# sharph/s-rack

Measured on AMD Instinct MI355X. Metric: voice-samples/sec @48 kHz offline render, higher is better.
Workload: dtype f32

## Files before the change

s-rack_amd/csrc/chain.hip:

```cpp
#include "fused.hip.h"
#include "launch.hpp"

namespace srack {

__global__ __launch_bounds__(64) void render_ctl_gate_env(CtlWork w)
{
    if (w.port & OSC_EXACT)
        ctl_gate_env<true>(w);
    else
        ctl_gate_env<false>(w);
}

void launch_ctl_gate_env(const CtlWork& w, hipStream_t st)
{
    hipLaunchKernelGGL(render_ctl_gate_env, dim3(1), dim3(64), 0, st, w);
}

void launch_fused(uint32_t osc_port, uint32_t vcf_port, bool exact, int out_mode, bool track, const KernelArgs& ka, const ChainRoles& roles, const CtlWork& co,
                  dim3 grid, hipStream_t st)
{
    with_osc_port(osc_port, [&](auto A) { launch_chain<decltype(A)::value>(vcf_port, exact, out_mode, track, ka, roles, co, grid, st); });
}

}
```

s-rack_amd/csrc/fused.hip.h:

```cpp
#pragma once
#include <hip/hip_runtime.h>
#include <type_traits>

#include "kernel_args.hip.h"
#include "launch_types.hpp"
#include "modules.hip.h"
#include "wave.hip.h"

#ifndef SRK_PRIO_AT1
#define SRK_PRIO_AT1 32
#endif
#ifndef SRK_PRIO_AT0
#define SRK_PRIO_AT0 56
#endif


namespace srack {


template <uint32_t kOscPort, bool kExact>
SRK_DEV void ctl_gate_env_body(const CtlWork& a)
{
    using namespace dev;
    const ChainRoles r{0, 0, 0, 1, 0, 2, 0};
    const int lane = threadIdx.x;
    auto row = [&](int rr) { return a.table[rr]; };
    const DevOp& ol = a.ops[r.osc_l];
    const DevOp& od = a.ops[r.adsr];
    float* __restrict__ track = a.track;

    COsc cl;
    cosc_init(cl, make_f64(row(ol.state_row + OSC_S_POS_LO), row(ol.state_row + OSC_S_POS_HI)), ol.delta);
    AdsrRegs sd;
    sd.phase = __uint_as_float(row(od.state_row + ADSR_S_PHASE));
    sd.mode = (int)row(od.state_row + ADSR_S_MODE);
    sd.r_val = __uint_as_float(row(od.state_row + ADSR_S_R_VAL));
    sd.from_a_val = __uint_as_float(row(od.state_row + ADSR_S_FROM_A));
    sd.gate_last = row(od.state_row + ADSR_S_GATE_LAST) != 0;
    const AdsrConst kd = adsr_consts(od.par_val[ADSR_P_A], od.par_val[ADSR_P_D], od.par_val[ADSR_P_S], od.par_val[ADSR_P_R], od.par_val[ADSR_P_SR]);
    AdsrSeg seg;
    adsr_seg_enter(sd, kd, seg);

    constexpr uint32_t osc_flags = OSC_AA | kOscPort | (kExact ? OSC_EXACT : 0u);
    for (uint32_t t0 = 0; t0 < a.T; t0 += kMixRows) {
        const int n = (int)min((uint32_t)kMixRows, a.T - t0);
        const float gate = cosc_tile<kExact>(osc_flags, cl, n);
        const float env = adsr_seg_tile(sd, kd, seg, gate, n);
        if (lane < n) track[t0 + lane] = env;
    }
    adsr_seg_flush(sd, seg);
    uint32_t* const tout = a.table_out ? a.table_out : a.table;
    if (a.table_out) {
        for (uint32_t rr = (uint32_t)lane; rr < a.n_rows; rr += 64u) a.table_out[rr] = a.table[rr];
        __builtin_amdgcn_fence(__ATOMIC_RELEASE, "workgroup");
    }
    if (lane == 0) {
        tout[ol.state_row + OSC_S_POS_LO] = f64_lo(cl.pos);
        tout[ol.state_row + OSC_S_POS_HI] = f64_hi(cl.pos);
        tout[ol.state_row + OSC_S_SYNC_LAST] = 0u;
        tout[od.state_row + ADSR_S_PHASE] = __float_as_uint(sd.phase);
        tout[od.state_row + ADSR_S_MODE] = (uint32_t)sd.mode;
        tout[od.state_row + ADSR_S_R_VAL] = __float_as_uint(sd.r_val);
        tout[od.state_row + ADSR_S_FROM_A] = __float_as_uint(sd.from_a_val);
        tout[od.state_row + ADSR_S_GATE_LAST] = sd.gate_last ? 1u : 0u;
    }
}


template <bool kExact>
SRK_DEV void ctl_gate_env(const CtlWork& w)
{
    const uint32_t port = w.port & (OSC_OUT_SINE | OSC_OUT_SQUARE | OSC_OUT_SAW);
    if (port == OSC_OUT_SQUARE)
        ctl_gate_env_body<OSC_OUT_SQUARE, kExact>(w);
    else if (port == OSC_OUT_SAW)
        ctl_gate_env_body<OSC_OUT_SAW, kExact>(w);
    else
        ctl_gate_env_body<OSC_OUT_SINE, kExact>(w);
}


template <uint32_t kOscAPort, uint32_t kOscLPort, uint32_t kVcfPort, bool kExact, int kOut>
__global__ __launch_bounds__(64) void render_voice_chain(KernelArgs a, ChainRoles r)
{
    using namespace dev;
    __shared__ __attribute__((aligned(16))) float mix_tile[kMixTile];
    const int lane = threadIdx.x;
    const WaveMap wm = wave_map(a, lane);
    const uint32_t voice = wm.voice, vc = wm.vc, V = a.V;
    const bool active = wm.active;
    auto row = [&](int rr) { return a.table[(size_t)rr * V + vc]; };
    auto parv = [&](const DevOp& op, int k) { return op.par_row[k] >= 0 ? __uint_as_float(row(op.par_row[k])) : op.par_val[k]; };

    const DevOp& oa = a.ops[r.osc_a];
    const DevOp& ol = a.ops[r.osc_l];
    const DevOp& ov = a.ops[r.vcf];
    const DevOp& od = a.ops[r.adsr];
    const DevOp& oc = a.ops[r.vca];
    const int plane = a.ops[r.out].aux;

    constexpr uint32_t kEx = kExact ? OSC_EXACT : 0u;
    constexpr uint32_t fa = OSC_AA | kOscAPort | kEx;
    constexpr uint32_t fl = OSC_AA | kOscLPort | kEx;

    OscRegs sa, sl;
    OscConst ka, kl;
    sa.pos = make_f64(row(oa.state_row + OSC_S_POS_LO), row(oa.state_row + OSC_S_POS_HI));
    sa.sync_last = row(oa.state_row + OSC_S_SYNC_LAST) != 0;
    sl.pos = make_f64(row(ol.state_row + OSC_S_POS_LO), row(ol.state_row + OSC_S_POS_HI));
    sl.sync_last = row(ol.state_row + OSC_S_SYNC_LAST) != 0;
    ka.sr = oa.sample_rate;
    ka.val = 0.0;
    ka.delta = oa.delta_row >= 0 ? make_f64(row(oa.delta_row), row(oa.delta_row + 1)) : oa.delta;
    ka.inv_dt = inv_dt_f32(ka.delta);
    kl.sr = ol.sample_rate;
    kl.val = 0.0;
    kl.delta = ol.delta_row >= 0 ? make_f64(row(ol.delta_row), row(ol.delta_row + 1)) : ol.delta;
    kl.inv_dt = inv_dt_f32(kl.delta);

    VcfRegs sv;
    {
        const int s0 = ov.state_row;
        sv.f = __uint_as_float(row(s0 + VCF_S_F));
        sv.p = __uint_as_float(row(s0 + VCF_S_P));
        sv.q = __uint_as_float(row(s0 + VCF_S_Q));
        sv.b0 = __uint_as_float(row(s0 + VCF_S_B0 + 0));
        sv.b1 = __uint_as_float(row(s0 + VCF_S_B0 + 1));
        sv.b2 = __uint_as_float(row(s0 + VCF_S_B0 + 2));
        sv.b3 = __uint_as_float(row(s0 + VCF_S_B0 + 3));
        sv.b4 = __uint_as_float(row(s0 + VCF_S_B0 + 4));
        sv.freq = __uint_as_float(row(s0 + VCF_S_FREQ));
// ... 99 lines not shown
        put(s0 + VCF_S_P, __float_as_uint(sv.p));
        put(s0 + VCF_S_Q, __float_as_uint(sv.q));
        put(s0 + VCF_S_B0 + 0, __float_as_uint(sv.b0));
        put(s0 + VCF_S_B0 + 1, __float_as_uint(sv.b1));
        put(s0 + VCF_S_B0 + 2, __float_as_uint(sv.b2));
        put(s0 + VCF_S_B0 + 3, __float_as_uint(sv.b3));
        put(s0 + VCF_S_B0 + 4, __float_as_uint(sv.b4));
        put(s0 + VCF_S_FREQ, __float_as_uint(sv.freq));
        put(s0 + VCF_S_RES, __float_as_uint(sv.res));
        put(od.state_row + ADSR_S_PHASE, __float_as_uint(sd.phase));
        put(od.state_row + ADSR_S_MODE, (uint32_t)sd.mode);
        put(od.state_row + ADSR_S_R_VAL, __float_as_uint(sd.r_val));
        put(od.state_row + ADSR_S_FROM_A, __float_as_uint(sd.from_a_val));
        put(od.state_row + ADSR_S_GATE_LAST, sd.gate_last ? 1u : 0u);
    }
}

#ifdef SRK_WAVE_CENSUS
static __device__ uint32_t* srk_census_rec;
SRK_DEV uint32_t* census_begin(uint32_t slot, uint32_t wave, bool ctl, int lane)
{
    uint32_t* rec = srk_census_rec;
    if (!rec || lane != 0) return nullptr;
    rec += (size_t)slot * 8;
    const uint64_t t = __builtin_amdgcn_s_memrealtime();
    rec[0] = (uint32_t)t;
    rec[1] = (uint32_t)(t >> 32);
    rec[4] = (uint32_t)__builtin_amdgcn_s_getreg((31 << 11) | 4);
    rec[5] = (uint32_t)__builtin_amdgcn_s_getreg((31 << 11) | 20);
    rec[6] = ctl ? 3u : 1u;
    rec[7] = wave;
    return rec;
}
SRK_DEV void census_end(uint32_t* rec)
{
    if (!rec) return;
    const uint64_t t = __builtin_amdgcn_s_memrealtime();
    rec[2] = (uint32_t)t;
    rec[3] = (uint32_t)(t >> 32);
}
SRK_DEV void census_end(uint32_t* rec, const dev::Pace& p)
{
    if (rec && p.word) rec[6] = 1u | 4u | (p.key << 3) | ((p.max_lead < 255u ? p.max_lead : 255u) << 16) | ((p.mine < 255u ? p.mine : 255u) << 24);
    census_end(rec);
}
#endif

template <uint32_t kOscAPort, uint32_t kVcfPort, bool kExact, int kOut>
__global__ __launch_bounds__(64) void render_voice_chain_track(KernelArgs a, ChainRoles r, CtlWork co)
{
    using namespace dev;
    __shared__ __attribute__((aligned(16))) float mix_tile[kMixTile];
    if (blockIdx.x < a.block0) {
        __builtin_amdgcn_s_setprio(3);
#ifdef SRK_WAVE_CENSUS
        uint32_t* crec = census_begin(a.n_waves, 0xffffffffu, true, threadIdx.x);
#endif
        ctl_gate_env<kExact>(co);
#ifdef SRK_WAVE_CENSUS
        census_end(crec);
#endif
        return;
    }
    const int lane = threadIdx.x;
#ifdef SRK_WAVE_CENSUS
    uint32_t* crec = census_begin(blockIdx.x - a.block0, blockIdx.x - a.block0, false, lane);
#endif
    const WaveMap wm = wave_map(a, lane);
    const uint32_t voice = wm.voice, vc = wm.vc, V = a.V;
    const bool active = wm.active;
    auto row = [&](int rr) { return a.table[(size_t)rr * V + vc]; };
    auto parv = [&](const DevOp& op, int k) { return op.par_row[k] >= 0 ? __uint_as_float(row(op.par_row[k])) : op.par_val[k]; };

    const DevOp& oa = a.ops[r.osc_a];
    const DevOp& ov = a.ops[r.vcf];
    const DevOp& oc = a.ops[r.vca];
    const int plane = a.ops[r.out].aux;
    const float* __restrict__ env_track = a.tracks + (size_t)r.track * a.t_stride;

    constexpr uint32_t fa = OSC_AA | kOscAPort | (kExact ? OSC_EXACT : 0u);
    OscRegs sa;
    OscConst ka;
    sa.pos = make_f64(row(oa.state_row + OSC_S_POS_LO), row(oa.state_row + OSC_S_POS_HI));
    sa.sync_last = row(oa.state_row + OSC_S_SYNC_LAST) != 0;
    ka.sr = oa.sample_rate;
    ka.val = 0.0;
    ka.delta = oa.delta_row >= 0 ? make_f64(row(oa.delta_row), row(oa.delta_row + 1)) : oa.delta;
    ka.inv_dt = inv_dt_f32(ka.delta);

    VcfRegs sv;
    const int s0 = ov.state_row;
    sv.f = __uint_as_float(row(s0 + VCF_S_F));
    sv.p = __uint_as_float(row(s0 + VCF_S_P));
    sv.q = __uint_as_float(row(s0 + VCF_S_Q));
    sv.b0 = __uint_as_float(row(s0 + VCF_S_B0 + 0));
    sv.b1 = __uint_as_float(row(s0 + VCF_S_B0 + 1));
    sv.b2 = __uint_as_float(row(s0 + VCF_S_B0 + 2));
    sv.b3 = __uint_as_float(row(s0 + VCF_S_B0 + 3));
    sv.b4 = __uint_as_float(row(s0 + VCF_S_B0 + 4));
    sv.freq = __uint_as_float(row(s0 + VCF_S_FREQ));
    sv.res = __uint_as_float(row(s0 + VCF_S_RES));
    if (a.T > 0) vcf_coeffs<!kExact>(sv, vcf_frequency(parv(ov, VCF_P_FREQ), 0.0f, parv(ov, VCF_P_EXP)), vcf_resonance(parv(ov, VCF_P_RES)));
    bool sv_fin = !kExact || vcf_nan_free(sv);
    const bool negative = parv(oc, VCA_P_NEG) != 0.0f;

    EmitOf<kOut> em = make_emit_of<kOut>(a, plane, lane);

    constexpr bool kFixed = !kExact && kOscAPort == OSC_OUT_SAW;
    COsc ca;
    FOsc fa_osc;
    float x = 0.0f;
// ... 155 lines not shown
```

s-rack_amd/csrc/launch_types.hpp:

```cpp
#pragma once
#include <cstdint>

#include "kernel_args.hip.h"

namespace srack {

struct CtlWork {
    const DevOp* ops;
    uint32_t* table;
    float* track;
    uint32_t T;
    uint32_t port;
    uint32_t* table_out;
    uint32_t n_rows;
};

constexpr int kBlkVoices = 32, kBlkSlices = 16, kBlkPer = 16, kBlkChunk = kBlkSlices * kBlkPer;

struct MasterArgs {
    const float* rows;
    const float* gain;
    float* runs;
    float* master;
    double* stats;
    uint32_t n;
    uint32_t n_buses;
    uint32_t row_channels;
    uint32_t used;
};

struct SendRun {
    uint32_t dst;
    uint32_t first;
    uint32_t count;
    int32_t srow;
};
struct SendMulti {
    uint32_t dst;
    uint32_t first_row;
    uint32_t n_runs;
    uint32_t pad;
};
static_assert(sizeof(SendRun) == 16 && sizeof(SendMulti) == 16, "the host keeps both tables as four 32-bit words per entry (runtime.hpp)");
struct SendArgs {
    const float* rows;
    float* out;
    float* scratch;
    const uint32_t* term_src;
    const float* term_gain;
    const SendRun* runs;
    const SendMulti* multi;
    uint32_t n;
    uint32_t row_channels;
    uint32_t used;
    uint32_t n_runs;
    uint32_t n_multi;
    uint32_t max_blocks;
};

struct BusVcfRow {
    uint32_t row;
    uint32_t bus;
    uint32_t slot;
    uint32_t port;
    float freq, res, exp_amt;
    uint32_t pad;
};
// ... 71 lines not shown
```

s-rack_amd/csrc/modules.hip.h:

```cpp
#pragma once
#ifndef __HIPCC_RTC__
#include <hip/hip_runtime.h>
#endif

#ifdef __HIPCC_RTC__
#include "srack_hip.h"
#else
#include "../../include/srack_hip.h"
#endif
#include "program.hpp"

namespace srack {
namespace dev {

#define SRK_DEV __device__ __forceinline__

SRK_DEV float keep(float x)
{
    asm("" : "+v"(x));
    return x;
}

SRK_DEV float zero_f32()
{
// ... 710 lines not shown
    uint64_t near = __builtin_amdgcn_ballot_w64(h <= o.hA) | __builtin_amdgcn_ballot_w64(h >= o.hB);
    if (kPort == OSC_OUT_SQUARE) near |= __builtin_amdgcn_ballot_w64((uint32_t)(h - o.hQ0) <= o.hQspan);
    if (near != 0) {
        OscRegs g;
        g.pos = o.pos;
        g.sync_last = false;
        OscConst k;
        k.delta = o.delta;
        k.val = 0.0;
        k.sr = 0.0;
        k.inv_dt = 0.0f;
        float o3[3] = {0.0f, 0.0f, 0.0f};
        osc_step(OSC_AA | OSC_EXACT | kPort, g, k, 0.0f, 0.0f, o3[0], o3[1], o3[2]);
        o.pos = g.pos;
        return kPort == OSC_OUT_SQUARE ? o3[1] : o3[2];
    }
    const float y = kPort == OSC_OUT_SQUARE ? (h < 0x3fe00000 ? -1.0f : 1.0f) : (float)o.pos * 2.0f - 1.0f;
    o.pos = __builtin_amdgcn_fract(o.pos + o.delta);
    return y;
}

template <bool kExact>
SRK_DEV float cosc_tile(uint32_t flags, COsc& o, int n)
{
    const int lane = (int)(threadIdx.x & 63u);
    double pos = o.pos, mine = o.pos;
    const bool tame = !kExact || __builtin_amdgcn_ballot_w64(!(pos >= 0.0 && pos < 1.0 && o.delta >= 0.0 && o.delta < 1.0)) == 0;
    if (tame && n == kTileRows) {
#pragma unroll 8
        for (int j = 0; j < kTileRows; j++) {
            mine = lane == j ? pos : mine;
            pos = __builtin_amdgcn_fract(pos + o.delta);
        }
    } else {
        for (int j = 0; j < n; j++) {
            mine = lane == j ? pos : mine;
            pos = tame ? __builtin_amdgcn_fract(pos + o.delta) : fmod1(pos + o.delta);
        }
    }
    o.pos = pos;
    OscRegs g;
    g.pos = mine;
    g.sync_last = false;
    OscConst k;
    k.delta = o.delta;
    k.val = 0.0;
    k.sr = 0.0;
    k.inv_dt = o.inv_dt;
    float y0 = 0.0f, y1 = 0.0f, y2 = 0.0f;
    osc_step(flags, g, k, 0.0f, 0.0f, y0, y1, y2);
    return (flags & OSC_OUT_SAW) ? y2 : ((flags & OSC_OUT_SQUARE) ? y1 : y0);
}

struct StepOsc {
    COsc o;
    float seen_cv;
    bool carried;
};

SRK_DEV void steposc_init(StepOsc& s, double pos)
{
    s.o.pos = pos;
    s.o.delta = 0.0;
    s.seen_cv = __builtin_nanf("");
    s.carried = false;
}

template <uint32_t kPort>
SRK_DEV float steposc_step(StepOsc& s, const OscConst& k, float cv)
{
    COsc& o = s.o;
    if (__builtin_amdgcn_ballot_w64(cv != s.seen_cv) != 0) {
        const double delta = osc_delta_cold((double)cv + k.val, k.sr);
        s.seen_cv = cv;
        s.carried = __builtin_amdgcn_ballot_w64(!(delta < 0.25)) == 0;
        cosc_init(o, o.pos, delta);
    }
    if (s.carried) return cosc_step<kPort>(o);
    OscRegs g;
    g.pos = o.pos;
    g.sync_last = false;
    g.seen_cv = s.seen_cv;
    g.seen_delta = o.delta;
    float o3[3] = {0.0f, 0.0f, 0.0f};
    osc_step(OSC_HAS_CV | OSC_CV_STEPWISE | OSC_AA | kPort, g, k, cv, 0.0f, o3[0], o3[1], o3[2]);
    cosc_init(o, g.pos, o.delta);
    return kPort == OSC_OUT_SAW ? o3[2] : (kPort == OSC_OUT_SQUARE ? o3[1] : o3[0]);
}

struct FOsc {
    uint32_t lo, hi;
    uint32_t dlo, dhi;
    float c32;
    float ta;
    float inv_s;
    bool first;
};

SRK_DEV void fosc_init(FOsc& o, uint32_t lo, uint32_t hi, uint32_t dlo, uint32_t dhi)
{
    o.lo = lo;
    o.hi = hi;
    o.dlo = dlo;
    o.dhi = dhi;
    const double delta = __builtin_fma((double)dhi, 0x1p-32, (double)dlo * 0x1p-64);
    o.inv_s = inv_dt_f32(delta) * 0x1p-32f;
// ... 414 lines not shown
    const bool open = g.c0 >= 0.0f && g.c1 >= 0.0f && (g.c0 > 0.0f || (g.c1 > 1.0e-30f && u_first > 1.0e-6f)) && g.c0 < 1.0e30f && g.c1 < 1.0e30f;
    decided = open || closed;
    return open;
}
SRK_DEV float vca_step_decided(bool open_lane, float audio, float cv)
{
    const float y = audio * cv;
    return open_lane ? y : 0.0f;
}

SRK_DEV float adsr_seg_quiet_step(AdsrRegs& s, AdsrSeg& g)
{
    s.phase = s.phase + g.inc;
    const float u = __builtin_fmaf(g.k1, s.phase, g.k0);
    const float out = g.c0 + g.c1 * u;
    g.held = out;
    return out;
}

SRK_DEV float adsr_seg_tile(AdsrRegs& s, const AdsrConst& c, AdsrSeg& g, float gate, int n)
{
    const int lane = (int)(threadIdx.x & 63u);
    const uint64_t tile = (1ull << n) - 1ull;
    const uint64_t high = __builtin_amdgcn_ballot_w64(gate > 0.0f) & tile;
    const uint64_t before = (high << 1) | (g.last != 0 ? 1ull : 0ull);
    float keep = 0.0f;
    int i = 0;
    while (i < n) {
        const uint64_t ends = ((g.on_high != 0 ? high : 0ull) | (g.on_low != 0 ? ~high : 0ull) | (g.on_edge != 0 ? (high & ~before) : 0ull)) & tile & (~0ull << i);
        const int by_gate = ends != 0 ? (int)__builtin_ctzll(ends) : n;
        const float room = (0.9999f - s.phase) * __builtin_amdgcn_rcpf(g.inc);
        const int by_phase = __builtin_amdgcn_readfirstlane(room > 0.0f ? (int)__builtin_fminf(room, 64.0f) : 0);
        const int run = min(by_gate - i, by_phase);
        if (run > 0) {
            float ph = s.phase, out = g.held;
            for (int k = 0; k < run; k++) {
                ph = ph + g.inc;
                const float u = __builtin_fmaf(g.k1, ph, g.k0);
                out = g.c0 + g.c1 * u;
                keep = lane == i + k ? out : keep;
            }
            s.phase = ph;
            g.held = out;
            i += run;
            g.last = ((high >> (i - 1)) & 1ull) ? ~0ull : 0ull;
        }
        if (i < n) {
            const float y = adsr_seg_step(s, c, g, __int_as_float(__builtin_amdgcn_readlane(__float_as_int(gate), i)));
            keep = lane == i ? y : keep;
            i++;
        }
    }
    return keep;
}

SRK_DEV float vca_step(uint32_t flags, bool negative, float audio, float cv)
{
    if ((flags & (VCA_HAS_AUDIO | VCA_HAS_CV)) != (VCA_HAS_AUDIO | VCA_HAS_CV)) return zero_f32();
    return (negative || cv > 0.0f) ? audio * cv : 0.0f;
}

SRK_DEV float vca_step_uniform(uint32_t flags, bool negative, float audio, float cv)
{
    if ((flags & (VCA_HAS_AUDIO | VCA_HAS_CV)) != (VCA_HAS_AUDIO | VCA_HAS_CV)) return zero_f32();
    const bool cv_pos = (uint32_t)(__float_as_int(cv) - 1) < 0x7f800000u;
    return (negative || cv_pos) ? audio * cv : 0.0f;
}

SRK_DEV float mixer_step(uint32_t connected, const float in[4], const float gain[4])
{
    float out = zero_f32();
#pragma unroll
    for (int k = 0; k < 4; k++)
        if (connected & (1u << k)) out = out + in[k] * gain[k];
    return out;
}

SRK_DEV float math_step(uint32_t flags, float in1, float in2, float constant)
{
    float a = (flags & MATH_HAS_IN1) ? in1 : zero_f32();
    float b = (flags & MATH_HAS_IN2) ? in2 : constant;
    switch ((flags >> MATH_OP_SHIFT) & 3u) {
    case SRACK_MATH_ADD: return a + b;
    case SRACK_MATH_SUBTRACT: return a - b;
    default: return a * b;
    }
}

SRK_DEV uint64_t splitmix64(uint64_t x)
{
    x += 0x9E3779B97F4A7C15ull;
    x = (x ^ (x >> 30)) * 0xBF58476D1CE4E5B9ull;
    x = (x ^ (x >> 27)) * 0x94D049BB133111EBull;
    return x ^ (x >> 31);
}
SRK_DEV uint64_t noise_voice_key(uint64_t base, uint64_t global_voice) { return splitmix64(base ^ global_voice); }
SRK_DEV float noise_sample(uint64_t key, uint64_t n)
{
    const uint32_t k24 = (uint32_t)(splitmix64(key + n * 0x9E3779B97F4A7C15ull) >> 40);
    return ((float)k24 * 0x1p-24f - 0.5f) * 2.0f;
}

__device__ const uint64_t kPowfLog2Tab[16][2] = {
    {0x3ff661ec79f8f3be, 0xbfdefec65b963019}, {0x3ff571ed4aaf883d, 0xbfdb0b6832d4fca4}, {0x3ff49539f0f010b0, 0xbfd7418b0a1fb77b},
    {0x3ff3c995b0b80385, 0xbfd39de91a6dcf7b}, {0x3ff30d190c8864a5, 0xbfd01d9bf3f2b631}, {0x3ff25e227b0b8ea0, 0xbfc97c1d1b3b7af0},
    {0x3ff1bb4a4a1a343f, 0xbfc2f9e393af3c9f}, {0x3ff12358f08ae5ba, 0xbfb960cbbf788d5c}, {0x3ff0953f419900a7, 0xbfaa6f9db6475fce},
// ... 213 lines not shown
```

s-rack_amd/csrc/render.hip:

```cpp
#include <hip/hip_runtime.h>

#include <algorithm>
#include <cstdio>
#include <cstdlib>
#include <cstring>
#include <memory>
#include <string>
#include <type_traits>
#include <vector>

#include "folds.hip.h"
#include "jit.hpp"
#include "kernel_args.hip.h"
#include "launch.hpp"
#include "runtime.hpp"
#include "wave.hip.h"

namespace srack {


struct Knobs {
    uint32_t want_waves = 1024;
    uint32_t chunk_max = 4096;
    uint32_t chunk_first = 1024;
    bool debug_occ = false;
    int high_prio_ctl = 1;
    int special_ctl = 1;
    int fm_split = 1;
    int fm_block = 1;
    uint32_t fm_block_chunk = 65536;
    uint32_t fm_block_min = 4096;
    int mix_aside = 0;
    int pace = 1;
    int tile_plain = 1;
    int tick = 2;
};
static const Knobs& knobs()
{
    static const Knobs k = [] {
        Knobs v;
        auto num = [](const char* name, long lo, long hi, long dflt) {
            const char* e = getenv(name);
            if (!e || !*e) return dflt;
            char* end = nullptr;
            const long x = strtol(e, &end, 10);
            if (end == e) return dflt;
            return std::min(std::max(x, lo), hi);
        };
        v.want_waves = (uint32_t)num("SRACK_WANT_WAVES", 1, 1 << 20, 1024);
        v.chunk_max = (uint32_t)num("SRACK_CHUNK_MAX", 256, 65536, 4096);
        v.chunk_first = (uint32_t)num("SRACK_CHUNK_FIRST", 32, 4096, 1024);
        v.debug_occ = getenv("SRACK_DEBUG_OCC") != nullptr;
        v.high_prio_ctl = (int)num("SRACK_CTL_HIGH_PRIO", 0, 1, 1);
        v.special_ctl = (int)num("SRACK_SPECIAL_CTL", 0, 1, 1);
        v.fm_split = (int)num("SRACK_FM_SPLIT", 0, 1, 1);
        v.fm_block = (int)num("SRACK_FM_BLOCK", 0, 1, 1);
        v.fm_block_chunk = (uint32_t)num("SRACK_FM_BLOCK_CHUNK", 256, 65536, 65536);
        v.fm_block_min = (uint32_t)num("SRACK_FM_BLOCK_MIN", 1, 65536, 4096);
        v.tick = (int)num("SRACK_TICK", 0, 2, 2);
        v.mix_aside = (int)num("SRACK_MIX_ASIDE", 0, 1, 0);
        v.pace = (int)num("SRACK_PACE", 0, 1, 1);
        v.tile_plain = (int)num("SRACK_TILE_PLAIN", 0, 1, 1);
        return v;
    }();
    return k;
}

struct DevProg {
    DevOp* d_ops = nullptr;
    uint32_t* d_table = nullptr;
    float* d_rings = nullptr;
    uint32_t* d_seqtab = nullptr;
    double* d_fv = nullptr;
    void release()
    {
        (void)hipFree(d_fv);
        d_fv = nullptr;
        (void)hipFree(d_ops);
        (void)hipFree(d_table);
        (void)hipFree(d_rings);
        (void)hipFree(d_seqtab);
        d_seqtab = nullptr;
        d_ops = nullptr;
        d_table = nullptr;
        d_rings = nullptr;
    }
};

struct TickSession {
    bool on = false;
    uint32_t L = 0;
    uint32_t Lmax = 0;
    uint32_t S = 0;
    uint32_t n = 0;
    uint32_t R = 0;
    uint64_t c = 0;
    uint64_t n0 = 0;
    hipStream_t st = nullptr;
    hipEvent_t done = nullptr;
    float* d_ring = nullptr;
    size_t ring_bytes = 0;
    std::vector<uint32_t*> d_copies;
    std::vector<size_t> words;
    uint64_t slots_base = 0;
    uint32_t slots_n = 0;
};
constexpr uint32_t kPaceSlices = 16;
constexpr uint32_t kTickBatch = 256, kTickFirstBatch = 8;

struct DeviceState {
    TickSession tick;
    hipStream_t mix_stream = nullptr;
    std::vector<hipEvent_t> ev_mix;
    hipEvent_t ev_mix_done = nullptr;
    DevProg voice;
// ... 379 lines not shown
    p.chunk = p.whole_segment ? k.fm_block_chunk : (p.kernel == Kernel::FmPairX || (fm_z1 && !general)) ? std::min(k.chunk_max, 2048u) : k.chunk_max;
    p.stats_in_kernel = p.kernel == Kernel::VoiceChain || p.kernel == Kernel::VoiceChainTrack;
    p.paced = p.kernel == Kernel::VoiceChainTrack && k.pace;
    return p;
}

static int resolve_specialized(PatchHandle& h, KernelPick& pick, uint32_t flags, int out_mode, const JitKernel** out, bool* with_ctl)
{
    *out = nullptr;
    *with_ctl = false;
    const FlatProgram& P = h.prog.voice;
    DeviceState* d = h.dev;
    if (!pick.candidate) return SRACK_OK;
    const bool forced = (flags & SRACK_RENDER_SPECIALIZE) != 0;
    if (!forced && (P.n_voices < kSpecializeMinVoices || d->jit_failed || !jit_supported(P))) return SRACK_OK;
    const bool ctl = h.prog.n_tracks > 0 && knobs().special_ctl && jit_ctl_supported(h.prog);
    const uint32_t n_waves = (P.n_voices + pick.lanes - 1) / pick.lanes;
    if (!d->jit[out_mode]) {
        JitFetchInfo how;
        const int rc = jit_get(h.prog, out_mode, ctl, &d->jit[out_mode], &how, (int)std::min(4u, (n_waves + 1023u) / 1024u));
        if (rc != SRACK_OK) {
            if (forced) return rc;
            d->jit_note = std::string(" jit=unavailable(") + last_error() + ")";
            if (d->jit_note.size() > 160) d->jit_note = d->jit_note.substr(0, 157) + "...)";
            for (char& c : d->jit_note)
                if (c == '\n') c = ' ';
            fprintf(stderr, "[srack] no specialised kernel for this program (%s): rendering through the pre-built kernels\n", last_error());
            d->jit_failed = true;
            return SRACK_OK;
        }
        char note[160];
        char budget[40] = "";
        if (how.waves > 0) std::snprintf(budget, sizeof budget, " regs=%d(budget for %d waves)", how.vgprs, how.waves);
        if (how.how == 2)
            std::snprintf(note, sizeof note, " jit=compiled(%.0f ms)%s", how.compile_ms, budget);
        else
            std::snprintf(note, sizeof note, " jit=%s%s", how.how == 1 ? "disk-cache" : "memory-cache", budget);
        d->jit_note = note;
        d->bank_lds[out_mode] = how.bank_lds;
    }
    d->last_bank_lds = d->bank_lds[out_mode];
    *out = d->jit[out_mode].get();
    *with_ctl = ctl;
    pick.name = "render_specialized";
    pick.stats_in_kernel = pick.paced = false;
    if (P.hdr.n_rings == 0 && n_waves <= 1024 && !(flags & SRACK_RENDER_EXACT_OSC)) pick.chunk = std::min(knobs().chunk_max, 2048u);
    return SRACK_OK;
}

static void launch_ctl(const FlatProgram& Cp, const KernelArgs& kc, hipStream_t st)
{
    if (Cp.fused == FUSED_CTL_GATE_ENV) {
        CtlWork w{kc.ops, kc.table, kc.frames + (size_t)Cp.ops[2].aux * kc.plane_stride, kc.T,
                  Cp.ops[0].flags & (OSC_OUT_SINE | OSC_OUT_SQUARE | OSC_OUT_SAW | OSC_EXACT), nullptr, 0u};
        launch_ctl_gate_env(w, st);
    } else if (Cp.fused == FUSED_FM_PAIR) {
        const bool exact = (Cp.render_flags & SRACK_RENDER_EXACT_OSC) != 0;
        launch_fm_pair(fm_pair_kernel(Cp.fused_variant, exact), exact, 1, kc, fm_pair_roles(Cp), dim3(1), st);
    } else {
        launch_interp(Cp, kc, st, knobs().debug_occ);
    }
}

#ifdef SRK_WAVE_CENSUS
static struct {
    uint32_t* d_rec = nullptr;
    uint32_t cap = 0, used = 0;
    std::vector<uint32_t> slots;
    std::vector<uint32_t*> where;
} g_census;

static uint32_t* const kCensusNone = nullptr;
uint32_t* const* census_rec = &kCensusNone;

static int census_arm(uint32_t n_slots)
{
    uint32_t* p = nullptr;
    if (g_census.d_rec && g_census.used + n_slots <= g_census.cap && g_census.where.size() < g_census.where.capacity()) {
        p = g_census.d_rec + (size_t)g_census.used * 8;
        g_census.used += n_slots;
        g_census.slots.push_back(n_slots);
    }
    census_rec = &kCensusNone;
    if (g_census.where.size() == g_census.where.capacity()) return SRACK_OK;
    g_census.where.push_back(p);
    census_rec = &g_census.where.back();
    return SRACK_OK;
}

extern "C" int srack_census_begin(uint32_t max_slots, uint32_t max_launches)
{
    HIP_TRY(hipDeviceSynchronize());
    (void)hipFree(g_census.d_rec);
    g_census = {};
    census_rec = &kCensusNone;
    HIP_TRY(hipMalloc(&g_census.d_rec, sizeof(uint32_t) * 8 * (size_t)max_slots));
    HIP_TRY(hipMemset(g_census.d_rec, 0, sizeof(uint32_t) * 8 * (size_t)max_slots));
    g_census.cap = max_slots;
    g_census.where.reserve(max_launches);
    HIP_TRY(hipDeviceSynchronize());
    return SRACK_OK;
}

extern "C" int srack_census_read(uint32_t* out, uint32_t max_slots, uint32_t* slots_per_launch, uint32_t max_launches)
{
    HIP_TRY(hipDeviceSynchronize());
    const uint32_t n = std::min<uint32_t>((uint32_t)g_census.slots.size(), max_launches);
    uint32_t words = 0;
    for (uint32_t i = 0; i < n; i++) {
        if (words / 8 + g_census.slots[i] > max_slots) return (int)i;
        slots_per_launch[i] = g_census.slots[i];
        words += 8 * g_census.slots[i];
    }
    if (words) HIP_TRY(hipMemcpy(out, g_census.d_rec, sizeof(uint32_t) * words, hipMemcpyDeviceToHost));
    g_census.where.clear();
    g_census.where.shrink_to_fit();
    return (int)n;
}
#endif

struct Segment {
    PatchHandle& h;
    const FlatProgram& P;
    DeviceState* const d;
    TickSession& tk;
    const uint32_t V, C, T_total, t_seg, T, flags;
    float *d_frames, *d_mix;
    double* d_stats;
    bool fold = false;
    uint32_t fold_rows = 0;
    float* d_bus;
    uint32_t bus_slab = 0;
    const hipStream_t st;
    int rc = SRACK_OK;
    KernelPick pick;
    const uint32_t lanes, n_waves;
    bool has_ctl = false, co_ctl = false, special_ctl = false, tick = false;
    uint32_t n_stages = 0, n_tracks = 0, kChunkMax = 0, kChunkFirst = 0, max_lag = 0, n_chunks = 0, n_ctl_launch = 0;
    uint32_t stride = 0;
    const JitKernel* special = nullptr;
    std::vector<std::pair<uint32_t, uint32_t>> chunks;
    ChainRoles roles{};
    SeqRoles seq{};
    uint32_t osc_port = 0, vcf_port = 0, seq_port = 0;
    MixArgs m{};
    bool mix_aside = false;

    Segment(PatchHandle& h_, uint32_t T_total_, uint32_t t_seg_, uint32_t T_, float* d_frames_, float* d_mix_, double* d_stats_, float* d_bus_, uint32_t flags_, hipStream_t st_)
        : h(h_), P(h_.prog.voice), d(h_.dev), tk(h_.dev->tick), V(h_.prog.voice.n_voices), C((uint32_t)h_.prog.voice.hdr.n_channels), T_total(T_total_),
          t_seg(t_seg_), T(T_), flags(flags_), d_frames(d_frames_ ? d_frames_ + (size_t)t_seg_ * h_.prog.voice.n_voices : nullptr),
          d_mix(d_mix_ ? d_mix_ + t_seg_ : nullptr), d_stats(d_stats_), d_bus(d_bus_ ? d_bus_ + t_seg_ : nullptr), st(st_), pick(pick_kernel(h_.prog, flags_, T_)), lanes(pick.lanes), n_waves((h_.prog.voice.n_voices + lanes - 1) / lanes)
    {
    }

    CtlWork ctl_work(uint32_t t_off, uint32_t len)
    {
        const FlatProgram& Cp = h.prog.ctl[0];
        return CtlWork{d->ctl[0].d_ops, d->ctl[0].d_table, d->d_tracks + (size_t)Cp.ops[2].aux * T + t_off, len,
                       Cp.ops[0].flags & (OSC_OUT_SINE | OSC_OUT_SQUARE | OSC_OUT_SAW | OSC_EXACT), nullptr, 0u};
    }
    int get_event(hipEvent_t& e)
    {
        if (!d->pool.empty()) {
            e = d->pool.back();
            d->pool.pop_back();
            return SRACK_OK;
        }
        HIP_TRY(hipEventCreate(&e));
        return SRACK_OK;
    }

    KernelArgs unit_args(uint32_t s)
    {
        KernelArgs kc{};
        kc.ops = d->ctl[s].d_ops;
        kc.prog = h.prog.ctl[s].hdr;
        kc.seqtab = d->ctl[s].d_seqtab;
        kc.V = 1;
        kc.n_waves = 1;
        kc.lanes = 64;
        kc.block0 = s;
        return kc;
    }
    KernelArgs stage_args(uint32_t s, uint32_t k)
    {
        const uint32_t t_off = chunks[k].first, len = chunks[k].second;
        KernelArgs kc = unit_args(s);
        kc.table = d->ctl[s].d_table;
        kc.rings = d->ctl[s].d_rings;
        kc.fv = d->ctl[s].d_fv;
        kc.frames = d->d_tracks + t_off;
        kc.tracks = d->d_tracks + t_off;
        kc.plane_stride = T;
        kc.t_stride = T;
        kc.T = len;
        kc.n0 = h.samples_rendered + t_off;
        return kc;
    }
    int upload_slots(hipStream_t on)
    {
        const size_t bytes = sizeof(KernelArgs) * d->h_stage_slots.size();
        if (bytes > d->stage_slots_cap) {
            (void)hipFree(d->d_stage_slots);
            d->d_stage_slots = nullptr;
            d->stage_slots_cap = 0;
            HIP_TRY(hipMalloc(&d->d_stage_slots, bytes));
            d->stage_slots_cap = bytes;
        }
        HIP_TRY(hipMemcpyAsync(d->d_stage_slots, d->h_stage_slots.data(), bytes, hipMemcpyHostToDevice, on));
        return SRACK_OK;
    }
    int upload_stage_slots(hipStream_t on)
    {
        d->h_stage_slots.assign((size_t)n_ctl_launch * n_stages, KernelArgs{});
        for (uint32_t s2 = 0; s2 < n_stages; s2++)
            for (uint32_t k = 0; k < n_chunks; k++) d->h_stage_slots[(size_t)(k + (uint32_t)h.prog.ctl_lag[s2]) * n_stages + s2] = stage_args(s2, k);
        return upload_slots(on);
    }
    float* tick_tracks(uint64_t x)
    {
        return tk.d_ring + (size_t)(x % tk.R) * tk.Lmax;
    }
    uint32_t tick_len(uint64_t x)
    {
        const uint32_t k = (uint32_t)(x % tk.n);
        return std::min(tk.Lmax, tk.L - k * tk.Lmax);
    }
    uint64_t tick_n0(uint64_t x)
    {
        return tk.n0 + (x / tk.n) * tk.L + (x % tk.n) * (uint64_t)tk.Lmax;
    }
    uint32_t* tick_table(uint32_t s2, uint64_t x)
    {
        if (tk.words[s2] == 0) return nullptr;
        return x == 0 ? d->ctl[s2].d_table : tk.d_copies[s2] + (size_t)(x % tk.R) * tk.words[s2];
    }
    KernelArgs tick_unit_args(uint32_t s2, uint64_t x)
    {
        KernelArgs kc = unit_args(s2);
        kc.table = tick_table(s2, x);
        kc.table_out = tick_table(s2, x + 1);
        kc.frames = tick_tracks(x);
        kc.tracks = kc.frames;
        kc.plane_stride = tk.S;
        kc.t_stride = tk.S;
        kc.T = tick_len(x);
        kc.n0 = tick_n0(x);
        return kc;
    }
    CtlWork tick_work(uint64_t x)
    {
        const FlatProgram& Cp = h.prog.ctl[0];
        return CtlWork{d->ctl[0].d_ops, tick_table(0, x), tick_tracks(x) + (size_t)Cp.ops[2].aux * tk.S, tick_len(x),
                       Cp.ops[0].flags & (OSC_OUT_SINE | OSC_OUT_SQUARE | OSC_OUT_SAW | OSC_EXACT), tick_table(0, x + 1), (uint32_t)Cp.hdr.n_rows};
    }
    int tick_upload_slots(uint64_t base)
    {
        const uint32_t fill = max_lag + 1, batch = std::max(base == 0 ? kTickFirstBatch : kTickBatch, tk.n);
        d->h_stage_slots.assign((size_t)(fill + batch) * n_stages, KernelArgs{});
        for (uint32_t s2 = 0; s2 < n_stages; s2++) {
            const uint32_t lag = (uint32_t)h.prog.ctl_lag[s2];
            if (base == 0)
                for (uint32_t g = lag; g < fill; g++) d->h_stage_slots[(size_t)g * n_stages + s2] = tick_unit_args(s2, g - lag);
            for (uint32_t i = 0; i < batch; i++) d->h_stage_slots[(size_t)(fill + i) * n_stages + s2] = tick_unit_args(s2, base + i + fill - lag);
        }
        if ((rc = upload_slots(st)) != SRACK_OK) return rc;
        tk.slots_base = base;
        tk.slots_n = batch;
        return SRACK_OK;
    }
    int bus_upload()
    {
        const BusPlan& B = h.bus_plan;
        if (d->d_bus_tab && d->bus_revision == h.bus_revision) return SRACK_OK;
        std::vector<uint32_t> w;
        auto put = [&w](const void* p, size_t n) { w.insert(w.end(), (const uint32_t*)p, (const uint32_t*)p + n); };
        put(h.bus_gain.data(), h.bus_gain.size());
        put(B.order.data(), B.order.size());
        put(B.tile_seg.data(), B.tile_seg.size());
        put(B.seg_end.data(), B.seg_end.size());
        put(B.seg_dst.data(), B.seg_dst.size());
        put(B.bus_first.data(), B.bus_first.size());
        put(B.bus_count.data(), B.bus_count.size());
        (void)hipFree(d->d_bus_tab);
        d->d_bus_tab = nullptr;
        HIP_TRY(hipMalloc(&d->d_bus_tab, sizeof(uint32_t) * w.size()));
        HIP_TRY(hipMemcpy(d->d_bus_tab, w.data(), sizeof(uint32_t) * w.size(), hipMemcpyHostToDevice));
        d->bus_revision = h.bus_revision;
        return SRACK_OK;
    }
    BusFoldArgs bus_args(const float* frames, uint64_t plane_stride, uint32_t t_at, uint32_t rows)
    {
        const BusPlan& B = h.bus_plan;
        BusFoldArgs b{};
        b.frames = frames;
        b.plane_stride = plane_stride;
        b.V = V;
        b.T = rows;
        const uint32_t* w = d->d_bus_tab;
        b.gain = (const float*)w;
        b.order = (w += h.bus_gain.size());
        b.tile_seg = (w += B.order.size());
        b.seg_end = (w += B.tile_seg.size());
        b.seg_dst = (const int32_t*)(w += B.seg_end.size());
        b.bus_first = (w += B.seg_dst.size());
        b.bus_count = (const int32_t*)(w += B.bus_first.size());
        b.part = d->d_bus_part;
// ... 242 lines not shown
        mix_aside = d_mix && n_chunks > 1 && knobs().mix_aside;
        if (mix_aside) {
            if (!d->mix_stream) HIP_TRY(hipStreamCreateWithFlags(&d->mix_stream, hipStreamNonBlocking));
            if (!d->ev_mix_done) HIP_TRY(hipEventCreateWithFlags(&d->ev_mix_done, hipEventDisableTiming));
            while (d->ev_mix.size() < n_chunks) {
                hipEvent_t e = nullptr;
                HIP_TRY(hipEventCreateWithFlags(&e, hipEventDisableTiming));
                d->ev_mix.push_back(e);
            }
        }
        const bool paced = pick.paced, exact = (flags & SRACK_RENDER_EXACT_OSC) != 0;
        if (paced && !d->d_pace) HIP_TRY(hipMalloc(&d->d_pace, sizeof(uint32_t) * dev::kPaceKeys * kPaceSlices));
        for (uint32_t k = 0; k < n_chunks; k++) {
            const uint32_t t_off = chunks[k].first, len = chunks[k].second;
            KernelArgs ka{};
            if (paced) {
                if (k % kPaceSlices == 0)
                    HIP_TRY(hipMemsetAsync(d->d_pace, 0, sizeof(uint32_t) * dev::kPaceKeys * std::min(kPaceSlices, n_chunks - k), st));
                ka.pace = d->d_pace + (size_t)(k % kPaceSlices) * dev::kPaceKeys;
            }
            ka.ops = d->voice.d_ops;
            ka.prog = P.hdr;
            ka.table = d->voice.d_table;
            ka.rings = d->voice.d_rings;
            ka.seqtab = d->voice.d_seqtab;
            ka.fv = d->voice.d_fv;
            ka.frames = d_frames ? d_frames + (size_t)t_off * V : nullptr;
            ka.mixpart = d_mix ? d->d_mixpart + t_off : nullptr;
            ka.tracks = tick ? tick_tracks(tk.c + k) : has_ctl ? d->d_tracks + t_off : nullptr;
            ka.plane_stride = (uint64_t)T_total * V;
            ka.t_stride = stride;
            ka.V = V;
            ka.T = len;
            ka.n_waves = n_waves;
            ka.lanes = lanes;
            ka.n0 = h.samples_rendered + t_off;
            ka.stats = fold ? nullptr : d_stats;
            ka.tile_plain = (uint32_t)knobs().tile_plain;
            if (fold_rows) {
                ka.frames = d->d_stat_frames;
                ka.plane_stride = (uint64_t)fold_rows * V;
            }
            CtlWork co{};
            if (tick && co_ctl) {
                co = tick_work(tk.c + k + 1);
                ka.block0 = 1;
            } else if (tick) {
                ka.block0 = n_stages;
                ka.ctl_slots = d->d_stage_slots + (size_t)(max_lag + 1 + (tk.c + k - tk.slots_base)) * n_stages;
            } else if (co_ctl && k + 1 < n_chunks) {
                co = ctl_work(chunks[k + 1].first, chunks[k + 1].second);
                ka.block0 = 1;
            }
            if (has_ctl && !co_ctl && !(special && special_ctl)) HIP_TRY(hipStreamWaitEvent(st, d->ev_chunk[k], 0));
            if (!tick && special && special_ctl && k + max_lag + 1 < n_ctl_launch) {
                ka.block0 = n_stages;
                ka.ctl_slots = d->d_stage_slots + (size_t)(k + max_lag + 1) * n_stages;
            }
            hipEvent_t e0 = nullptr, e1 = nullptr;
            const bool timed = h.timing_armed;
            if (timed) {
                if ((rc = get_event(e0)) != SRACK_OK || (rc = get_event(e1)) != SRACK_OK) return rc;
                HIP_TRY(hipEventRecord(e0, st));
            }
            const int out_mode = (ka.frames ? 1 : 0) | (ka.mixpart ? 2 : 0);
            if (special) {
                if ((rc = jit_launch(*special, ka, n_waves + ka.block0, st)) != SRACK_OK) return rc;
            } else {
                switch (pick.kernel) {
                case Kernel::VoiceChainTrack:
#ifdef SRK_WAVE_CENSUS
                    if ((rc = census_arm(n_waves + 1)) != SRACK_OK) return rc;
#endif
                    [[fallthrough]];
                case Kernel::VoiceChain:
                    launch_fused(osc_port, vcf_port, exact, out_mode | (ka.stats ? kOutStats : 0), pick.kernel == Kernel::VoiceChainTrack, ka, roles, co, dim3(n_waves + ka.block0), st);
                    break;
                case Kernel::SeqChain: launch_seq(seq_port, out_mode, ka, seq, dim3(n_waves), st); break;
                case Kernel::FmPairX: launch_fm_pair_x(out_mode, ka, roles, dim3(n_waves), st); break;
                case Kernel::FmPairBlock:
                case Kernel::FmPairBlockX:
                    HIP_TRY(launch_fm_block(pick.kernel == Kernel::FmPairBlockX, out_mode, ka, roles, st));
                    break;
                case Kernel::FmPair:
                case Kernel::FmPairRing:
                case Kernel::FmPairSplit: launch_fm_pair(pick.kernel, exact, out_mode, ka, roles, dim3(n_waves), st); break;
                case Kernel::Interp: launch_interp(P, ka, st, knobs().debug_occ); break;
                }
            }
            HIP_TRY(hipGetLastError());
            if (fold) {
                hipLaunchKernelGGL(stats_fold, dim3((V + 255) / 256, (uint32_t)P.hdr.n_planes), dim3(256), 0, st, ka.frames, ka.plane_stride, V, len, d_stats);
                HIP_TRY(hipGetLastError());
            }
            if (d_bus) {
                const uint32_t n_seg = (uint32_t)h.bus_plan.seg_end.size();
                for (uint32_t r0 = 0; r0 < len; r0 += bus_slab) {
                    const uint32_t rows = std::min(bus_slab, len - r0);
                    const BusFoldArgs b = bus_args(ka.frames + (size_t)r0 * V, ka.plane_stride, t_off + r0, rows);
                    if (n_seg > 0) hipLaunchKernelGGL(bus_fold_tiles, dim3(h.bus_plan.n_tiles, (rows + kBusRows - 1) / kBusRows, (uint32_t)P.hdr.n_planes), dim3(64), 0, st, b);
                    hipLaunchKernelGGL(bus_fold_sum, dim3(h.n_buses * ((rows + 255) / 256)), dim3(256), 0, st, b);
                    HIP_TRY(hipGetLastError());
                }
            }
            if (mix_aside && k + 1 < n_chunks) {
                HIP_TRY(hipEventRecord(d->ev_mix[k], st));
// ... 186 lines not shown
```

s-rack_amd/csrc/wave.hip.h:

```cpp
#pragma once
#ifndef __HIPCC_RTC__
#include <hip/hip_runtime.h>
#endif

#include "kernel_args.hip.h"
#include "modules.hip.h"

#ifndef SRK_FRAME_AUX
#define SRK_FRAME_AUX 2
#endif


namespace srack {

namespace dev {

SRK_DEV double make_f64(uint32_t lo, uint32_t hi) { return __hiloint2double((int)hi, (int)lo); }
SRK_DEV uint32_t f64_lo(double d) { return (uint32_t)__double2loint(d); }
SRK_DEV uint32_t f64_hi(double d) { return (uint32_t)__double2hiint(d); }

SRK_DEV float readlane_f32(float v, int lane) { return __int_as_float(__builtin_amdgcn_readlane(__float_as_int(v), lane)); }

SRK_DEV bool track_flat(const float* p, int lane)
{
// ... 39 lines not shown
struct Pace {
    uint32_t* word;
    uint32_t mine;
#ifdef SRK_WAVE_CENSUS
    uint32_t key, max_lead;
#endif
};

SRK_DEV uint32_t pace_key()
{
    const uint32_t hw = (uint32_t)__builtin_amdgcn_s_getreg((31 << 11) | 4);
    const uint32_t xcc = (uint32_t)__builtin_amdgcn_s_getreg((31 << 11) | 20);
    return ((xcc & 7u) << 10) | (((hw >> 8) & 0xffu) << 2) | ((hw >> 4) & 3u);
}

SRK_DEV Pace pace_join(uint32_t* slice, int lane)
{
    Pace p{};
    if (!slice) return p;
    const uint32_t key = pace_key();
    p.word = slice + key;
    if (lane == 0) atomicAdd(p.word, kPaceMember);
#ifdef SRK_WAVE_CENSUS
    p.key = key;
#endif
    return p;
}

SRK_DEV bool pace_step(Pace& p, uint32_t tile, int lane, uint32_t& seen)
{
    seen = 0u;
    if (!p.word || tile == 0u || tile % SRK_PACE_TILES != 0u) return false;
    p.mine++;
    if (lane == 0) seen = atomicAdd(p.word, 1u);
    return true;
}

SRK_DEV void pace_apply(Pace& p, uint32_t seen)
{
    const uint32_t got = (uint32_t)__builtin_amdgcn_readfirstlane((int)seen);
    const int n = (int)(got >> 24);
    const int lead = n * (int)p.mine - (int)((got & (kPaceMember - 1u)) + 1u);
    const int band = SRK_PACE_LEAD * (n > 2 ? n - 1 : 1);
    if (lead >= band)
        __builtin_amdgcn_s_setprio(0);
    else if (lead <= -band)
        __builtin_amdgcn_s_setprio(2);
    else
        __builtin_amdgcn_s_setprio(1);
#ifdef SRK_WAVE_CENSUS
    const uint32_t al = (uint32_t)(lead < 0 ? -lead : lead);
    p.max_lead = al > p.max_lead ? al : p.max_lead;
#endif
}

}

constexpr int kMixRows = 32;
static_assert(kMixRows == dev::kTileRows, "the tile-wise module forms (modules.hip.h) assume the mix tile's length");
constexpr int kMixPitch = 68;
constexpr int kMixTile = kMixRows * kMixPitch;

constexpr int kStatCount = 6;
enum { kStatSum = 0, kStatSumSq = 1, kStatPeakPos = 2, kStatPeakNeg = 3, kStatNonfinite = 4, kStatClipped = 5 };

struct VoiceStats {
    double sum, sum_sq;
    float peak_pos, peak_neg;
    uint32_t nonfinite, clipped;
};

SRK_DEV void stats_add(VoiceStats& s, float x)
{
    const bool fin = __builtin_isfinite(x);
    const float xs = fin ? x : -0.0f;
    const double xd = (double)xs;
    s.sum += xd;
    s.sum_sq = __builtin_fma(xd, xd, s.sum_sq);
    s.peak_pos = xs > s.peak_pos ? xs : s.peak_pos;
    s.peak_neg = -xs > s.peak_neg ? -xs : s.peak_neg;
    s.nonfinite += fin ? 0u : 1u;
    s.clipped += fabsf(xs) > 1.0f ? 1u : 0u;
}

SRK_DEV void stats_load(VoiceStats& s, const double* p, size_t V)
{
    s.sum = p[(size_t)kStatSum * V];
    s.sum_sq = p[(size_t)kStatSumSq * V];
    s.peak_pos = (float)p[(size_t)kStatPeakPos * V];
    s.peak_neg = (float)p[(size_t)kStatPeakNeg * V];
    s.nonfinite = s.clipped = 0u;
}
SRK_DEV void stats_store(const VoiceStats& s, double* p, size_t V)
{
    p[kStatSum * V] = s.sum;
    p[kStatSumSq * V] = s.sum_sq;
    p[kStatPeakPos * V] = (double)s.peak_pos;
    p[kStatPeakNeg * V] = (double)s.peak_neg;
    p[kStatNonfinite * V] += (double)s.nonfinite;
    p[kStatClipped * V] += (double)s.clipped;
}

struct Emit {
    float* frame_row;
    __amdgpu_buffer_rsrc_t rsrc;
    uint32_t soff;
// ... 175 lines not shown
```

Measured before the change: 1255 billion.

## Add DPP lane-shift gate/env tile path and optional paced control-wave yielding

```diff
diff --git a/s-rack_amd/csrc/chain.hip b/s-rack_amd/csrc/chain.hip
--- a/s-rack_amd/csrc/chain.hip
+++ b/s-rack_amd/csrc/chain.hip
@@ -5,10 +5,11 @@
 
 __global__ __launch_bounds__(64) void render_ctl_gate_env(CtlWork w)
 {
+    dev::CtlYield alone{};
     if (w.port & OSC_EXACT)
-        ctl_gate_env<true>(w);
+        ctl_gate_env<true>(w, alone);
     else
-        ctl_gate_env<false>(w);
+        ctl_gate_env<false>(w, alone);
 }
 
 void launch_ctl_gate_env(const CtlWork& w, hipStream_t st)
diff --git a/s-rack_amd/csrc/fused.hip.h b/s-rack_amd/csrc/fused.hip.h
--- a/s-rack_amd/csrc/fused.hip.h
+++ b/s-rack_amd/csrc/fused.hip.h
@@ -19,7 +19,7 @@
 
 
 template <uint32_t kOscPort, bool kExact>
-SRK_DEV void ctl_gate_env_body(const CtlWork& a)
+SRK_DEV void ctl_gate_env_body(const CtlWork& a, dev::CtlYield& yield)
 {
     using namespace dev;
     const ChainRoles r{0, 0, 0, 1, 0, 2, 0};
@@ -44,9 +44,16 @@
     constexpr uint32_t osc_flags = OSC_AA | kOscPort | (kExact ? OSC_EXACT : 0u);
     for (uint32_t t0 = 0; t0 < a.T; t0 += kMixRows) {
         const int n = (int)min((uint32_t)kMixRows, a.T - t0);
-        const float gate = cosc_tile<kExact>(osc_flags, cl, n);
-        const float env = adsr_seg_tile(sd, kd, seg, gate, n);
-        if (lane < n) track[t0 + lane] = env;
+        ctl_yield_tile(yield, t0 / kMixRows, (a.T + (uint32_t)kMixRows - 1u) / (uint32_t)kMixRows, lane);
+        if (n == kMixRows && cosc_tile_tame<kExact>(cl)) {
+            const float gate = cosc_tile_shift<kExact>(osc_flags, cl);
+            const float env = adsr_seg_tile_shift(sd, kd, seg, gate);
+            if (lane < kMixRows) track[t0 + (uint32_t)(kMixRows - 1 - lane)] = env;
+        } else {
+            const float gate = cosc_tile<kExact>(osc_flags, cl, n);
+            const float env = adsr_seg_tile(sd, kd, seg, gate, n);
+            if (lane < n) track[t0 + lane] = env;
+        }
     }
     adsr_seg_flush(sd, seg);
     uint32_t* const tout = a.table_out ? a.table_out : a.table;
@@ -68,15 +75,15 @@
 
 
 template <bool kExact>
-SRK_DEV void ctl_gate_env(const CtlWork& w)
+SRK_DEV void ctl_gate_env(const CtlWork& w, dev::CtlYield& yield)
 {
     const uint32_t port = w.port & (OSC_OUT_SINE | OSC_OUT_SQUARE | OSC_OUT_SAW);
     if (port == OSC_OUT_SQUARE)
-        ctl_gate_env_body<OSC_OUT_SQUARE, kExact>(w);
+        ctl_gate_env_body<OSC_OUT_SQUARE, kExact>(w, yield);
     else if (port == OSC_OUT_SAW)
-        ctl_gate_env_body<OSC_OUT_SAW, kExact>(w);
+        ctl_gate_env_body<OSC_OUT_SAW, kExact>(w, yield);
     else
-        ctl_gate_env_body<OSC_OUT_SINE, kExact>(w);
+        ctl_gate_env_body<OSC_OUT_SINE, kExact>(w, yield);
 }
 
 
@@ -282,11 +289,11 @@
     using namespace dev;
     __shared__ __attribute__((aligned(16))) float mix_tile[kMixTile];
     if (blockIdx.x < a.block0) {
-        __builtin_amdgcn_s_setprio(3);
+        CtlYield yield = ctl_yield_begin(co.yield != 0u ? a.pace : nullptr, a.T);
 #ifdef SRK_WAVE_CENSUS
         uint32_t* crec = census_begin(a.n_waves, 0xffffffffu, true, threadIdx.x);
 #endif
-        ctl_gate_env<kExact>(co);
+        ctl_gate_env<kExact>(co, yield);
 #ifdef SRK_WAVE_CENSUS
         census_end(crec);
 #endif
diff --git a/s-rack_amd/csrc/launch_types.hpp b/s-rack_amd/csrc/launch_types.hpp
--- a/s-rack_amd/csrc/launch_types.hpp
+++ b/s-rack_amd/csrc/launch_types.hpp
@@ -13,6 +13,7 @@
     uint32_t port;
     uint32_t* table_out;
     uint32_t n_rows;
+    uint32_t yield;
 };
 
 constexpr int kBlkVoices = 32, kBlkSlices = 16, kBlkPer = 16, kBlkChunk = kBlkSlices * kBlkPer;
diff --git a/s-rack_amd/csrc/modules.hip.h b/s-rack_amd/csrc/modules.hip.h
--- a/s-rack_amd/csrc/modules.hip.h
+++ b/s-rack_amd/csrc/modules.hip.h
@@ -786,6 +786,46 @@
     return (flags & OSC_OUT_SAW) ? y2 : ((flags & OSC_OUT_SQUARE) ? y1 : y0);
 }
 
+#ifndef SRK_CTL_OSC_UNROLL
+#define SRK_CTL_OSC_UNROLL 32
+#endif
+SRK_DEV uint32_t lane_push(uint32_t hist, uint32_t v)
+{
+    return (uint32_t)__builtin_amdgcn_update_dpp((int)v, (int)hist, 0x138 , 0xf, 0xf, false);
+}
+SRK_DEV float lane_push(float hist, float v) { return __uint_as_float(lane_push(__float_as_uint(hist), __float_as_uint(v))); }
+
+template <bool kExact>
+SRK_DEV bool cosc_tile_tame(const COsc& o)
+{
+    return !kExact || __builtin_amdgcn_ballot_w64(!(o.pos >= 0.0 && o.pos < 1.0 && o.delta >= 0.0 && o.delta < 1.0)) == 0;
+}
+
+template <bool kExact>
+SRK_DEV float cosc_tile_shift(uint32_t flags, COsc& o)
+{
+    double pos = o.pos;
+    uint32_t lo = (uint32_t)__double2loint(pos), hi = (uint32_t)__double2hiint(pos);
+#pragma unroll SRK_CTL_OSC_UNROLL
+    for (int j = 0; j < kTileRows; j++) {
+        lo = lane_push(lo, (uint32_t)__double2loint(pos));
+        hi = lane_push(hi, (uint32_t)__double2hiint(pos));
+        pos = __builtin_amdgcn_fract(pos + o.delta);
+    }
+    o.pos = pos;
+    OscRegs g;
+    g.pos = __hiloint2double((int)hi, (int)lo);
+    g.sync_last = false;
+    OscConst k;
+    k.delta = o.delta;
+    k.val = 0.0;
+    k.sr = 0.0;
+    k.inv_dt = o.inv_dt;
+    float y0 = 0.0f, y1 = 0.0f, y2 = 0.0f;
+    osc_step(flags, g, k, 0.0f, 0.0f, y0, y1, y2);
+    return (flags & OSC_OUT_SAW) ? y2 : ((flags & OSC_OUT_SQUARE) ? y1 : y0);
+}
+
 struct StepOsc {
     COsc o;
     float seen_cv;
@@ -1306,6 +1346,42 @@
         }
     }
     return keep;
+}
+
+SRK_DEV float adsr_seg_tile_shift(AdsrRegs& s, const AdsrConst& c, AdsrSeg& g, float gate_rev)
+{
+    constexpr int n = kTileRows;
+    const uint64_t tile = (1ull << n) - 1ull;
+    const uint64_t high = (uint64_t)__builtin_bitreverse32((uint32_t)__builtin_amdgcn_ballot_w64(gate_rev > 0.0f));
+    const uint64_t before = (high << 1) | (g.last != 0 ? 1ull : 0ull);
+    float hist = 0.0f;
+    int i = 0;
+    while (i < n) {
+        const uint64_t ends = ((g.on_high != 0 ? high : 0ull) | (g.on_low != 0 ? ~high : 0ull) | (g.on_edge != 0 ? (high & ~before) : 0ull)) & tile & (~0ull << i);
+        const int by_gate = ends != 0 ? (int)__builtin_ctzll(ends) : n;
+        const float room = (0.9999f - s.phase) * __builtin_amdgcn_rcpf(g.inc);
+        const int by_phase = __builtin_amdgcn_readfirstlane(room > 0.0f ? (int)__builtin_fminf(room, 64.0f) : 0);
+        const int run = min(by_gate - i, by_phase);
+        if (run > 0) {
+            float ph = s.phase, out = g.held;
+            for (int k = 0; k < run; k++) {
+                ph = ph + g.inc;
+                const float u = __builtin_fmaf(g.k1, ph, g.k0);
+                out = g.c0 + g.c1 * u;
+                hist = lane_push(hist, out);
+            }
+            s.phase = ph;
+            g.held = out;
+            i += run;
+            g.last = ((high >> (i - 1)) & 1ull) ? ~0ull : 0ull;
+        }
+        if (i < n) {
+            const float y = adsr_seg_step(s, c, g, __int_as_float(__builtin_amdgcn_readlane(__float_as_int(gate_rev), n - 1 - i)));
+            hist = lane_push(hist, y);
+            i++;
+        }
+    }
+    return hist;
 }
 
 SRK_DEV float vca_step(uint32_t flags, bool negative, float audio, float cv)
diff --git a/s-rack_amd/csrc/render.hip b/s-rack_amd/csrc/render.hip
--- a/s-rack_amd/csrc/render.hip
+++ b/s-rack_amd/csrc/render.hip
@@ -33,6 +33,7 @@
     int mix_aside = 0;
     int pace = 1;
     int tile_plain = 1;
+    int ctl_yield = 0;
     int tick = 2;
 };
 static const Knobs& knobs()
@@ -61,6 +62,7 @@
         v.mix_aside = (int)num("SRACK_MIX_ASIDE", 0, 1, 0);
         v.pace = (int)num("SRACK_PACE", 0, 1, 1);
         v.tile_plain = (int)num("SRACK_TILE_PLAIN", 0, 1, 1);
+        v.ctl_yield = (int)num("SRACK_CTL_YIELD", 0, 1, Knobs().ctl_yield);
         return v;
     }();
     return k;
@@ -546,7 +548,7 @@
 {
     if (Cp.fused == FUSED_CTL_GATE_ENV) {
         CtlWork w{kc.ops, kc.table, kc.frames + (size_t)Cp.ops[2].aux * kc.plane_stride, kc.T,
-                  Cp.ops[0].flags & (OSC_OUT_SINE | OSC_OUT_SQUARE | OSC_OUT_SAW | OSC_EXACT), nullptr, 0u};
+                  Cp.ops[0].flags & (OSC_OUT_SINE | OSC_OUT_SQUARE | OSC_OUT_SAW | OSC_EXACT), nullptr, 0u, 0u};
         launch_ctl_gate_env(w, st);
     } else if (Cp.fused == FUSED_FM_PAIR) {
         const bool exact = (Cp.render_flags & SRACK_RENDER_EXACT_OSC) != 0;
@@ -651,7 +653,7 @@
     {
         const FlatProgram& Cp = h.prog.ctl[0];
         return CtlWork{d->ctl[0].d_ops, d->ctl[0].d_table, d->d_tracks + (size_t)Cp.ops[2].aux * T + t_off, len,
-                       Cp.ops[0].flags & (OSC_OUT_SINE | OSC_OUT_SQUARE | OSC_OUT_SAW | OSC_EXACT), nullptr, 0u};
+                       Cp.ops[0].flags & (OSC_OUT_SINE | OSC_OUT_SQUARE | OSC_OUT_SAW | OSC_EXACT), nullptr, 0u, 0u};
     }
     int get_event(hipEvent_t& e)
     {
@@ -746,7 +748,7 @@
     {
         const FlatProgram& Cp = h.prog.ctl[0];
         return CtlWork{d->ctl[0].d_ops, tick_table(0, x), tick_tracks(x) + (size_t)Cp.ops[2].aux * tk.S, tick_len(x),
-                       Cp.ops[0].flags & (OSC_OUT_SINE | OSC_OUT_SQUARE | OSC_OUT_SAW | OSC_EXACT), tick_table(0, x + 1), (uint32_t)Cp.hdr.n_rows};
+                       Cp.ops[0].flags & (OSC_OUT_SINE | OSC_OUT_SQUARE | OSC_OUT_SAW | OSC_EXACT), tick_table(0, x + 1), (uint32_t)Cp.hdr.n_rows, 0u};
     }
     int tick_upload_slots(uint64_t base)
     {
@@ -1095,6 +1097,7 @@
                 co = ctl_work(chunks[k + 1].first, chunks[k + 1].second);
                 ka.block0 = 1;
             }
+            co.yield = (uint32_t)knobs().ctl_yield;
             if (has_ctl && !co_ctl && !(special && special_ctl)) HIP_TRY(hipStreamWaitEvent(st, d->ev_chunk[k], 0));
             if (!tick && special && special_ctl && k + max_lag + 1 < n_ctl_launch) {
                 ka.block0 = n_stages;
diff --git a/s-rack_amd/csrc/wave.hip.h b/s-rack_amd/csrc/wave.hip.h
--- a/s-rack_amd/csrc/wave.hip.h
+++ b/s-rack_amd/csrc/wave.hip.h
@@ -115,6 +115,49 @@
     const uint32_t al = (uint32_t)(lead < 0 ? -lead : lead);
     p.max_lead = al > p.max_lead ? al : p.max_lead;
 #endif
+}
+
+#ifndef SRK_CTL_LEAD
+#define SRK_CTL_LEAD 8
+#endif
+
+struct CtlYield {
+    uint32_t* word;
+    uint32_t steps;
+    uint32_t seen;
+};
+
+SRK_DEV CtlYield ctl_yield_begin(uint32_t* slice, uint32_t T_voice)
+{
+    CtlYield y{};
+    y.steps = T_voice / ((uint32_t)kTileRows * SRK_PACE_TILES);
+    if (!slice || y.steps == 0u) {
+        __builtin_amdgcn_s_setprio(3);
+        return y;
+    }
+    y.word = slice + pace_key();
+    __builtin_amdgcn_s_setprio(0);
+    return y;
+}
+
+SRK_DEV void ctl_yield_tile(CtlYield& y, uint32_t tile, uint32_t tiles, int lane)
+{
+    if (!y.word) return;
+    if (tile > 1u && (tile - 1u) % SRK_PACE_TILES == 0u) {
+        const uint32_t got = (uint32_t)__builtin_amdgcn_readfirstlane((int)y.seen);
+        const int64_t members = (int64_t)(got >> 24), sum = (int64_t)(got & (kPaceMember - 1u));
+        if (members == 0) {
+            __builtin_amdgcn_s_setprio(3);
+        } else {
+            const int64_t lead = (int64_t)(tile - 1u) * members * (int64_t)y.steps - sum * (int64_t)tiles;
+            const int64_t band = (int64_t)SRK_CTL_LEAD * (int64_t)tiles * members * (int64_t)y.steps;
+            if (64 * lead >= band)
+                __builtin_amdgcn_s_setprio(0);
+            else if (128 * lead < band)
+                __builtin_amdgcn_s_setprio(3);
+        }
+    }
+    if (tile != 0u && tile % SRK_PACE_TILES == 0u && lane == 0) y.seen = atomicAdd(y.word, 0u);
 }
 
 }
```

Result: no change. 1256 billion (median of 2 runs) (+0.1%).
